# LMCache/LMCache

Measured on NVIDIA H100. Metric: kv_encode_decode_raw_GBps, higher is better.
Workload: dtype f32->u8 (bf16 KV)

## Files before the change

### lmcache_b200/csrc/codec.cu

```cuda
#include <cuda_bf16.h>
#include <cuda_fp16.h>
#include <cuda_runtime.h>
#include <stdint.h>
#include <stdlib.h>
#include <string.h>

#include <algorithm>
#include <vector>

#include "ac_core.cuh"
#include "common.cuh"

namespace b200kv {

constexpr int CT = 128;
constexpr int SPW = 6;
constexpr int SYMW = 43;
constexpr int PAIRW = 33;
constexpr int TEMPW_FUSED = 40;
constexpr int TEMPW_SPLIT = 132;
constexpr int TEMPW_FUSED_RANS = 48;
constexpr int CODER_AC = 0, CODER_RANS = 1;
constexpr int CODER_RANS_COMPACT = 2;
constexpr int kHdrRowWords = 8;
// ... 758 lines not shown
        const unsigned long long end = carry + wbase + inc;
        if (i < P.n_chunks) {
            const unsigned long long reserve = (end - start) * (unsigned long long)P.layers_left / (unsigned)P.nlay;
            const bool fits = (unsigned)i < fail0 && end + reserve <= (unsigned long long)P.arena_bytes;
            P.chunk_base[i] = fits ? end - v : ~0ull;
            if (fits) {
                P.ptotal[i] += P.totals[i];
                atomicMax(&s_end, end);
            } else {
                atomicOr(&P.err[i], 16u);
                atomicMin(&s_fail, (unsigned)i);
            }
        }
        __syncthreads();
        if (tid == 0) s_carry = s_end;
        __syncthreads();
    }
    if (tid == 0) {
        *P.cursor = s_carry;
        *P.fail_from = s_fail;
    }
    const int NLc = 2 * P.nlay;
    for (int k = tid; k < P.n_chunks * NLc; k += 1024) {
        const int j = k / NLc, pl = k - j * NLc;
        const uint32_t* tb = P.tile_tot + (int64_t)j * P.tiles_full;
        const unsigned long long off = tb[pl * P.tpp];
        const unsigned long long end = pl + 1 < NLc ? (unsigned long long)tb[(pl + 1) * P.tpp] : P.totals[j];
        const unsigned long long cb = P.chunk_base[j];
        int64_t* row = P.seg + ((int64_t)j * 2 * P.L + launch_plane(P, pl)) * 2;
        row[0] = cb == ~0ull ? -1 : (int64_t)(cb + off);
        row[1] = (int64_t)(end - off);
    }
}

__global__ void encl_init_kernel(EncParams P) {
    *P.cursor = 0ull;
    *P.fail_from = (unsigned)P.n_chunks;
}

__global__ void finalize_kernel(EncParams P) {
    const int j = blockIdx.x * blockDim.x + threadIdx.x;
    if (j >= P.n_chunks) return;
    const int t = chunk_tokens_of(P, j);
    const Layout lo = layout_of(P, t);
    b200kv_header* hd = reinterpret_cast<b200kv_header*>(P.out + (int64_t)j * P.out_stride);
    hd->magic = B200KV_MAGIC;
    hd->version = P.compact ? 3u : (uint32_t)P.coder + 1u;
    hd->L = P.L; hd->H = P.H; hd->D = P.D;
    hd->ntokens = t;
    hd->ngroups = lo.ngroups;
    hd->max_dtype = P.dtype;
    hd->payload_bytes = P.totals[j];
    hd->total_bytes = (uint64_t)lo.off_payload + P.totals[j];
    hd->status = P.err[j];
    hd->reserved[0] = hd->reserved[1] = hd->reserved[2] = 0u;
    if (P.sizes_out) P.sizes_out[j] = hd->status ? 0ull : hd->total_bytes;
    {
        uint8_t* c = reinterpret_cast<uint8_t*>(hd);
        const int64_t NL = 2 * (int64_t)P.L;
        const int64_t ends[3] = {lo.off_cdf + (P.compact ? NL : NL * P.C * kLp * 2), lo.off_maxes + NL * t * 2,
                                 lo.off_lengths + (int64_t)lo.ngroups * NL * P.C * (P.compact ? 1 : 4)};
        const int64_t starts[3] = {lo.off_maxes, lo.off_lengths, lo.off_payload};
        for (int k = 0; k < 3; ++k)
            for (int64_t b = ends[k]; b < starts[k]; ++b) c[b] = 0u;
    }
    if (P.compact) {
        uint8_t* nbmap = reinterpret_cast<uint8_t*>(hd) + lo.off_cdf;
        const int NL = 2 * P.L;
        for (int nl = 0; nl < (int)align16(NL); ++nl) nbmap[nl] = nl < NL ? (uint8_t)(2 * ((int)P.pt.maxq[nl] + 1)) : (uint8_t)0;
    }
}

struct DecChunk {
    const uint8_t* base;
    int64_t dst_tok;
    int32_t t, ngroups;
    uint32_t payload_bytes;
    int32_t ct0, ntw, cw0, cw1, dshift;
};

constexpr int kInlinePlanes = 128;
struct DecParams {
    PlaneTableT<kInlinePlanes> pt;
    const PlaneTable* gpt;
    int64_t sT, sH;
    const int64_t* slot_map;
    int32_t L, H, D, C, out_dtype, max_dtype, n_chunks, tpp, tiles_max;
    int32_t compact;
    int32_t lb, nlay;
    int32_t wtpp;
    const DecChunk* chunks;
    unsigned long long* tile_base;
    uint32_t* status;
};
static_assert(sizeof(DecParams) < kMaxParamBytes, "DecParams must stay under 4 KB of kernel parameters");

template <bool GT>
__device__ __forceinline__ const uint16_t* dec_plane(const DecParams& P, int nl) {
    if constexpr (GT) return P.gpt->p[nl];
    else return P.pt.p[nl];
}
template <bool GT>
__device__ __forceinline__ float dec_maxq(const DecParams& P, int nl) {
    if constexpr (GT) return P.gpt->maxq[nl];
    else return P.pt.maxq[nl];
}

__global__ void __launch_bounds__(128) tile_sum_kernel(DecParams P) {
    const int j = blockIdx.y;
    const int tile = blockIdx.x * 4 + (threadIdx.x >> 5);
    const int lane = threadIdx.x & 31;
    const DecChunk dc = P.chunks[j];
    const int NL = 2 * P.L;
    const int ntiles = dc.ngroups * NL * P.tpp;
    if (tile >= ntiles) return;
    const int plane_row = tile / P.tpp;
    const int ct = tile - plane_row * P.tpp;
    const Layout lo = layout_of(P, dc.t);
    const int c0 = ct * CT, c1 = min(P.C, c0 + CT);
    uint32_t s = 0;
    for (int c = c0 + lane; c < c1; c += 32) s += load_len(dc.base + lo.off_lengths, (int64_t)plane_row * P.C + c, P.compact != 0);
    s = __reduce_add_sync(0xffffffffu, s);
    if (lane == 0) P.tile_base[(int64_t)j * P.tiles_max + tile] = s;
}

__global__ void __launch_bounds__(1024) tile_scan_kernel(DecParams P) {
    __shared__ unsigned long long s_w[32];
    __shared__ unsigned long long s_carry;
    const int j = blockIdx.x;
    const DecChunk dc = P.chunks[j];
    const int ntiles = dc.ngroups * 2 * P.L * P.tpp;
    unsigned long long* tb = P.tile_base + (int64_t)j * P.tiles_max;
    const int lane = threadIdx.x & 31, wid = threadIdx.x >> 5;
    if (threadIdx.x == 0) s_carry = 0ull;
    __syncthreads();
    for (int base = 0; base < ntiles; base += 1024) {
        const int i = base + threadIdx.x;
        const unsigned long long v = i < ntiles ? tb[i] : 0ull;
        unsigned long long inc = v;
#pragma unroll
        for (int o = 1; o < 32; o <<= 1) {
            unsigned long long n = __shfl_up_sync(0xffffffffu, inc, o);
            if (lane >= o) inc += n;
        }
        if (lane == 31) s_w[wid] = inc;
        __syncthreads();
        unsigned long long wbase = 0ull, tot = 0ull;
        for (int w = 0; w < 32; ++w) {
            const unsigned long long s = s_w[w];
            if (w < wid) wbase += s;
            tot += s;
        }
        const unsigned long long carry = s_carry;
        if (i < ntiles) tb[i] = carry + wbase + inc - v;
        __syncthreads();
        if (threadIdx.x == 0) s_carry = carry + tot;
        __syncthreads();
    }
}

__global__ void __launch_bounds__(1024) plane_offsets_kernel(const uint8_t* base, int64_t stride, int64_t* out) {
    __shared__ uint32_t s_sum[B200KV_MAX_PLANES];
    const uint8_t* c = base + (int64_t)blockIdx.x * stride;
    int64_t* o = out + (int64_t)blockIdx.x * (B200KV_MAX_PLANES + 1);
    const uint32_t* hw = reinterpret_cast<const uint32_t*>(c);
    const uint32_t version = hw[1], L = hw[2], H = hw[3], D = hw[4], t = hw[5];
    const uint64_t total = *reinterpret_cast<const uint64_t*>(c + 40);
    const uint64_t C64 = (uint64_t)H * D;
    if (hw[0] != B200KV_MAGIC || version != 3u || L == 0u || 2u * L > (uint32_t)B200KV_MAX_PLANES || H == 0u || D == 0u ||
        t == 0u || t > (uint32_t)kGroup || C64 > (uint64_t)stride || C64 >= (1ull << 31)) {
        if (threadIdx.x == 0) o[0] = -1;
        return;
    }
    const int NL = 2 * (int)L;
    const int64_t C = (int64_t)C64;
    const Layout lo = make_layout((int)L, (int)C, (int)t, 1);
    if ((uint64_t)lo.off_payload > total || lo.off_payload > stride) {
        if (threadIdx.x == 0) o[0] = -1;
        return;
    }
    const uint8_t* half = c + lo.off_lengths;
    const int lane = threadIdx.x & 31, warp = threadIdx.x >> 5;
    for (int p = NL + 1 + (int)threadIdx.x; p <= B200KV_MAX_PLANES; p += blockDim.x) o[p] = 0;
    for (int p = warp; p < NL; p += blockDim.x >> 5) {
        const uint8_t* row = half + p * C;
        uint32_t sum = 0;
        if ((C & 15) == 0) {
            const uint4* v = reinterpret_cast<const uint4*>(row);
#pragma unroll 4
            for (int64_t i = lane; i < C / 16; i += 32) {
                const uint4 q = v[i];
                sum = __dp4a(q.x, 0x01010101u, sum);
                sum = __dp4a(q.y, 0x01010101u, sum);
                sum = __dp4a(q.z, 0x01010101u, sum);
                sum = __dp4a(q.w, 0x01010101u, sum);
            }
        } else {
            for (int64_t i = lane; i < C; i += 32) sum += row[i];
        }
        sum = __reduce_add_sync(0xffffffffu, sum);
        if (lane == 0) s_sum[p] = sum;
    }
    __syncthreads();
    if (threadIdx.x == 0) {
        int64_t off = lo.off_payload;
        o[0] = off;
        for (int p = 0; p < NL; ++p) {
            off += 2 * (int64_t)s_sum[p];
            o[p + 1] = off;
        }
        if (off != (int64_t)total) o[0] = -1;
    }
}

struct WordSrc {
    const uint32_t* base;
    uint32_t idx;
    uint32_t ahead;
    __device__ __forceinline__ void prime() { ahead = __ldg(base + idx); ++idx; }
    __device__ __forceinline__ uint32_t next_be() {
        const uint32_t w = ahead;
        ahead = __ldg(base + idx);
        ++idx;
        return __byte_perm(w, 0u, 0x0123);
    }
};

struct LeWordSrc {
    const uint32_t* p;
    __device__ __forceinline__ uint32_t next_le() { return __ldg(p++); }
};

__device__ __forceinline__ uint16_t out_half(float v, int dt) {
    return dt ? __half_as_ushort(__float2half_rn(v)) : __bfloat16_as_ushort(__float2bfloat16_rn(v));
}
template <int OUT_DT>
__device__ __forceinline__ void store_half(uint16_t* p, float v) {
    if constexpr (OUT_DT) *reinterpret_cast<__half*>(p) = __float2half_rn(v);
    else *reinterpret_cast<__nv_bfloat16*>(p) = __float2bfloat16_rn(v);
}

template <int OUT_DT>
__device__ __forceinline__ void store_dequant(uint16_t* base, uint32_t off, float lutv, float row_max, uint32_t two) {
    const float v = __fmul_rn(lutv, row_max);
    if constexpr (OUT_DT)
        asm volatile("{\n\t.reg .b64 ad;\n\t.reg .b32 r;\n\t.reg .b16 lo, hi;\n\t"
                     "mad.wide.u32 ad, %1, %3, %0;\n\t"
                     "cvt.rn.f16x2.f32 r, 0f00000000, %2;\n\t"
                     "mov.b32 {lo, hi}, r;\n\t"
                     "st.global.b16 [ad], lo;\n\t}" ::"l"(base), "r"(off), "f"(v), "r"(two) : "memory");
    else
        asm volatile("{\n\t.reg .b64 ad;\n\t.reg .b32 r;\n\t.reg .b16 lo, hi;\n\t"
                     "mad.wide.u32 ad, %1, %3, %0;\n\t"
                     "cvt.rn.bf16x2.f32 r, 0f00000000, %2;\n\t"
                     "mov.b32 {lo, hi}, r;\n\t"
                     "st.global.b16 [ad], lo;\n\t}" ::"l"(base), "r"(off), "f"(v), "r"(two) : "memory");
}

template <int OUT_DT, int NSTEPS, bool PAGED>
__device__ __forceinline__ void decode_stream(const uint8_t* cont, uint32_t my_off, const uint32_t* erow,
                                              const float* lut, const float* mx, uint16_t* dst, uint32_t sT, int gt,
                                              const int64_t* slots) {
    const uint32_t skip = my_off & 3u;
    WordSrc src{reinterpret_cast<const uint32_t*>(cont), my_off >> 2, 0u};
    src.prime();
    DecState2 st;
    dec_init2(st, src, skip);
    uint16_t* d = dst;
    auto lut_at = [&](uint32_t s4) { return *reinterpret_cast<const float*>(reinterpret_cast<const char*>(lut) + s4); };
    if constexpr (PAGED) {
        for (int i = 0; i < gt - 1; ++i)
            store_half<OUT_DT>(dst + __ldg(slots + i) * (int64_t)sT,
                               dequant_value(lut_at(dec_symbol2<NSTEPS>(st, src, erow, false)), mx[i]));
        store_half<OUT_DT>(dst + __ldg(slots + gt - 1) * (int64_t)sT,
                           dequant_value(lut_at(dec_symbol2<NSTEPS>(st, src, erow, true)), mx[gt - 1]));
    } else {
        for (int i = 0; i < gt - 1; ++i, d += sT)
            store_half<OUT_DT>(d, dequant_value(lut_at(dec_symbol2<NSTEPS>(st, src, erow, false)), mx[i]));
        store_half<OUT_DT>(d, dequant_value(lut_at(dec_symbol2<NSTEPS>(st, src, erow, true)), mx[gt - 1]));
    }
}

template <uint32_t ROWS, uint32_t PITCH>
__device__ __forceinline__ void rans_search_step(uint32_t& a, uint32_t key, uint32_t one) {
    uint32_t ev;
    asm volatile("ld.shared.u32 %0, [%1+%2];" : "=r"(ev) : "r"(a), "n"(ROWS * PITCH));
    asm("{\n\t.reg .pred p;\n\tsetp.le.u32 p, %1, %2;\n\t@p mad.lo.u32 %0, %3, %4, %0;\n\t}"
        : "+r"(a) : "r"(ev), "r"(key), "r"(one), "n"(ROWS * PITCH));
}

template <int OUT_DT, int NSTEPS, bool PAGED, bool TR>
__device__ __forceinline__ uint32_t rans_decode_stream(const uint8_t* cont, uint32_t my_off, const uint32_t* pk,
                                                       const float* lut, const float* mx, uint16_t* dst, uint32_t sT, int gt,
                                                       const int64_t* slots, uint32_t one) {
    const uint32_t* const wbase = reinterpret_cast<const uint32_t*>(cont);
    uint32_t idx = my_off >> 2;
    struct Src {
        const uint32_t* b; uint32_t& i;
        __device__ __forceinline__ uint32_t next_le() { return __ldg(b + i++); }
    } src{wbase, idx};
    RansDec st;
    rans_dec_init(st, src, (my_off >> 1) & 1u);
    constexpr uint32_t H = 1u << (NSTEPS - 1);
    constexpr uint32_t kPitch = TR ? CT * 4u : 4u;
    constexpr uint32_t kIdx = TR ? CT : 1u;
    const uint32_t a0 = (uint32_t)__cvta_generic_to_shared(pk);
    const uint32_t a0h = a0 + kPitch * H;
    const uint32_t r_mid = pk[kIdx * H], r_lo = pk[kIdx * (H / 2)], r_hi = pk[kIdx * (H + H / 2)];
    const uint32_t lut_a = (uint32_t)__cvta_generic_to_shared(lut);
    const uint32_t lut_rel = lut_a - a0;
    uint32_t off = 0u;
    const uint32_t c64k = one << 16, mone = 0u - one, two = one + one, c25 = one << 25;
    auto step = [&](float row_max, int i) {
        uint32_t key, xh;
        asm("mad.lo.u32 %0, %1, %2, 65535;" : "=r"(key) : "r"(st.x), "r"(c64k));
        asm("mul.hi.u32 %0, %1, %2;" : "=r"(xh) : "r"(st.x), "r"(c64k));
        const bool p1 = r_mid <= key;
        uint32_t a = p1 ? a0h : a0;
        const uint32_t m = p1 ? r_hi : r_lo;
        asm("{\n\t.reg .pred p;\n\tsetp.le.u32 p, %1, %2;\n\t@p mad.lo.u32 %0, %3, %4, %0;\n\t}"
            : "+r"(a) : "r"(m), "r"(key), "r"(one), "n"(kPitch * (H / 2)));
        if constexpr (H >= 16) rans_search_step<4, kPitch>(a, key, one);
        rans_search_step<2, kPitch>(a, key, one);
        rans_search_step<1, kPitch>(a, key, one);
        uint32_t e, la;
        float lv;
        asm volatile("ld.shared.u32 %0, [%1];" : "=r"(e) : "r"(a));
        if constexpr (TR) asm("mad.hi.u32 %0, %1, %2, %3;" : "=r"(la) : "r"(a - a0), "r"(c25), "r"(lut_a));
        else la = a + lut_rel;
        asm volatile("ld.shared.f32 %0, [%1];" : "=f"(lv) : "r"(la));
        uint32_t dl;
        asm("mul.hi.u32 %0, %1, %2;" : "=r"(dl) : "r"(key - e), "r"(c64k));
        st.x = (e & 0xffffu) * xh + dl;
        const uint32_t* const wad = wbase + idx;
        asm volatile(
            "{\n\t.reg .pred p, q;\n\t"
            "setp.lt.u32 p, %0, 65536;\n\t"
            "setp.eq.and.u32 q, %3, 0x1076, p;\n\t"
            "@p prmt.b32 %0, %0, %1, %3;\n\t"
            "@p mad.lo.u32 %3, %3, %7, 0x20ca;\n\t"
            "@q mov.b32 %1, %2;\n\t"
            "@q ld.global.nc.u32 %2, [%5];\n\t"
            "@q mad.lo.u32 %4, %6, %6, %4;\n\t"
            "}"
            : "+r"(st.x), "+r"(st.cur), "+r"(st.nxt), "+r"(st.sel), "+r"(idx)
            : "l"(wad), "r"(one), "r"(mone));
        if constexpr (PAGED) {
            store_dequant<OUT_DT>(dst + __ldg(slots + i) * (int64_t)sT, 0u, lv, row_max, two);
        } else {
            store_dequant<OUT_DT>(dst, off, lv, row_max, two);
            asm("mad.lo.u32 %0, %1, %2, %0;" : "+r"(off) : "r"(one), "r"(sT));
        }
    };
    int i = 0;
#pragma unroll 1
    for (; i + 4 <= gt; i += 4) {
        const float4 m4 = *reinterpret_cast<const float4*>(mx + i);
        step(m4.x, i); step(m4.y, i + 1); step(m4.z, i + 2); step(m4.w, i + 3);
    }
#pragma unroll 1
    for (; i < gt; ++i) step(mx[i], i);
    return st.x;
}

template <int OUT_DT, bool PAGED, int CODER, bool TR, bool GT>
__global__ void __launch_bounds__(CT, 12) decode_kernel(DecParams P) {
    extern __shared__ __align__(128) uint32_t smem[];
    uint32_t* tab = smem;
    float* mx = reinterpret_cast<float*>(smem + CT * kLp);
    float* lut = mx + kGroup;
    __shared__ uint32_t s_warp[CT / 32];

    const int tid = threadIdx.x;
    const int j = blockIdx.y;
    const DecChunk dc = P.chunks[j];
    const int NL = 2 * P.L;
    const int per_group = NL * P.tpp;
    const int launch_group = 2 * P.nlay * P.wtpp;
    const int g = blockIdx.x / launch_group;
    if (g >= dc.ngroups) return;
    const int kt = blockIdx.x - g * launch_group;
    const int kp = kt / P.wtpp;
    const int wt = kt - kp * P.wtpp;
    if (wt >= dc.ntw) return;
    const int nl = kp + (kp < P.nlay ? P.lb : P.L - P.nlay + P.lb);
    const int ct = dc.ct0 + wt;
    const int tile = g * per_group + nl * P.tpp + ct;
    const int tok0 = g * kGroup;
    const int gt = min(kGroup, dc.t - tok0);
    const int c = ct * CT + tid;
    const bool in_c = c < P.C;
    const bool active = c >= dc.cw0 && c < dc.cw1;
    const int ncols = min(CT, P.C - ct * CT);
    const Layout lo = layout_of(P, dc.t);

    const uint32_t len = in_c ? load_len(dc.base + lo.off_lengths, ((int64_t)g * NL + nl) * P.C + c, P.compact != 0) : 0u;
    uint32_t tile_total;
    const uint32_t my_rel = block_excl_scan(len, s_warp, &tile_total);
    const unsigned long long want = P.tile_base[(int64_t)j * P.tiles_max + tile] + my_rel;
    const bool beyond = want + len > (unsigned long long)dc.payload_bytes;
    const uint32_t my_off = (uint32_t)lo.off_payload + (uint32_t)min(want, (unsigned long long)dc.payload_bytes);

    const uint16_t* cdf_src = reinterpret_cast<const uint16_t*>(dc.base + lo.off_cdf) + ((int64_t)nl * P.C + ct * CT) * kLp;
    const uint16_t* maxes = reinterpret_cast<const uint16_t*>(dc.base + lo.off_maxes) + (int64_t)nl * dc.t + tok0;
    const float cq = dec_maxq<GT>(P, nl);
    bool built = false;
    uint32_t hl = 0u;
    if constexpr (CODER == CODER_RANS) {
        if (P.compact) {
            float* pn = mx;
            const float tf = (float)dc.t;
            for (int n = tid; n <= kGroup; n += CT) pn[n] = fdiv((float)n, tf);
            __syncthreads();
            const int nb = 2 * ((int)cq + 1);
            const uint32_t mbytes = (uint32_t)hdr_mask_bytes(nb);
            const uint8_t* sp = dc.base + my_off;
            const uint32_t al = (uint32_t)(reinterpret_cast<uintptr_t>(sp) & 3u);
            const uint32_t* wp = reinterpret_cast<const uint32_t*>(sp - al);
            const uint32_t fs = 8u * al;
            uint32_t x_prev = __ldg(wp), x_next = __ldg(wp + 1);
            const uint32_t hb0 = __funnelshift_r(x_prev, x_next, fs);
            uint32_t mask = hb0;
            if (nb <= 8) mask &= 0xffu;
            else if (nb <= 16) mask &= 0xffffu;
            if (nb < 32) mask &= (1u << nb) - 1u;
            hl = hdr_len(mask, nb);
            const uint32_t top = 0x80000000u >> __clz((int)mask);
            const bool all_short = __popc(__ballot_sync(0xffffffffu, active && hl > 8u)) < 8;
            const uint32_t wany = __reduce_or_sync(0xffffffffu, active ? mask : 0u);
            if (active) {
                uint32_t sum = 0u;
                uint32_t hb[9];
                uint32_t widx = mbytes >> 2, inw = mbytes & 3u, cur = 0u;
                const uint8_t* const cb = sp + mbytes;
                if (!all_short) {
                    hb[0] = hb0;
#pragma unroll
                    for (int k = 1; k < 9; ++k) {
                        hb[k] = 0u;
                        if ((uint32_t)(4 * k) < hl && (k < 5 || nb > 16)) {
                            x_prev = x_next;
                            x_next = __ldg(wp + k + 1);
                            hb[k] = __funnelshift_r(x_prev, x_next, fs);
                        }
                    }
                    cur = (widx == 0u ? hb[0] : hb[1]) >> (8u * inw);
                }
                auto next_byte = [&]() -> uint32_t {
                    const uint32_t v = cur & 255u;
                    cur >>= 8;
                    if (++inw == 4u) {
                        inw = 0u;
                        ++widx;
                        cur = hb[1];
#pragma unroll
                        for (int k = 2; k < 9; ++k) cur = widx == (uint32_t)k ? hb[k] : cur;
                    }
                    return v;
                };
                auto count = [&](int i) -> uint32_t {
                    if (i >= nb) return 0u;
                    const uint32_t bit = 1u << (i & 31);
                    uint32_t n = 0u;
                    if (all_short) {
                        const uint32_t below = i == 0 ? 0u : mask & (0xffffffffu >> (32 - (i & 31)));
                        const uint32_t v = __ldg(cb + __popc(below));
                        n = (mask & bit) ? v : 0u;
                        n = (top & bit) ? (uint32_t)dc.t - sum : n;
                        sum += n;
                    } else if (mask & bit) {
                        n = (top & bit) ? (uint32_t)dc.t - sum : next_byte();
                        sum += n;
                    }
                    return min(n, (uint32_t)kGroup);
                };
                CdfAccum2 acc;
                acc.init();
                uint32_t c0 = 0u;
                const int nsearch = cq <= 7.0f ? 16 : 32;
#pragma unroll
                for (int i = 0; i < 32; ++i) {
                    if (i < nsearch) {
                        if ((wany >> i) & 1u) acc.absorb(pn[count(i)]);
                        uint32_t c1 = acc.value((uint32_t)i + 1u);
                        if (i == 31) c1 = 0x10000u;
                        const uint32_t e = rans_table_entry(c0, c1);
                        if (TR) tab[i * CT + tid] = e;
                        else tab[tid * kLp + i] = e;
                        c0 = c1;
                    }
                }
            }
            __syncthreads();
            for (int i = tid; i < gt; i += CT) mx[i] = half_to_float(maxes[i], P.max_dtype);
            if (tid < 32) lut[tid] = dequant_lut((uint32_t)tid, cq);
            built = true;
        }
    }
    if (!built) {
        if constexpr (CODER == CODER_RANS && TR) {
            uint16_t* stg = reinterpret_cast<uint16_t*>(smem) + (CT * kLp);
            for (int e = tid; e < ncols * kLp; e += CT) stg[e] = __ldg(cdf_src + e);
            for (int i = tid; i < gt; i += CT) mx[i] = half_to_float(maxes[i], P.max_dtype);
            if (tid < 32) lut[tid] = dequant_lut((uint32_t)tid, cq);
            __syncthreads();
            const uint16_t* my = stg + tid * kLp;
            if (active) {
                uint32_t c0 = my[0];
    #pragma unroll
                for (int i = 0; i < 16; ++i) {
                    const uint32_t c1 = my[i + 1];
                    tab[i * CT + tid] = rans_table_entry(c0, c1);
                    c0 = c1;
                }
            }
            if (cq > 7.0f) {
                uint32_t cv[17];
                if (active) {
    #pragma unroll
                    for (int i = 0; i < 16; ++i) cv[i] = my[16 + i];
                    cv[16] = 0x10000u;
                }
                __syncthreads();
                if (active) {
    #pragma unroll
                    for (int i = 0; i < 16; ++i) tab[(16 + i) * CT + tid] = rans_table_entry(cv[i], cv[i + 1]);
                }
            }
        } else {
            for (int e = tid; e < ncols * kLp; e += CT) {
                const uint32_t i = (uint32_t)e % (uint32_t)kLp;
                const uint32_t c0 = __ldg(cdf_src + e);
                if constexpr (CODER == CODER_RANS) {
                    const uint32_t c1 = i < 31u ? (uint32_t)__ldg(cdf_src + e + 1) : 0x10000u;
                    tab[e] = i < 32u ? rans_table_entry(c0, c1) : 0xFFFFFFFFu;
                } else {
                    tab[e] = dec_table_entry(i, c0);
                }
            }
            for (int i = tid; i < gt; i += CT) mx[i] = half_to_float(maxes[i], P.max_dtype);
            if (tid < 32) lut[tid] = dequant_lut((uint32_t)tid, cq);
        }
    }
    __syncthreads();

    if (!active) return;
    const uint32_t* erow = tab + tid * kLp;
    const int oc = c + dc.dshift;
    const int h = oc / P.D;
    uint16_t* dst = const_cast<uint16_t*>(dec_plane<GT>(P, nl)) + (PAGED ? 0 : (dc.dst_tok + tok0) * P.sT) + (int64_t)h * P.sH +
                    (oc - h * P.D);
    const int64_t* slots = PAGED ? P.slot_map + dc.dst_tok + tok0 : nullptr;
    uint32_t bad = beyond ? 2u : 0u;
    if constexpr (CODER == CODER_RANS) {
        uint32_t xf;
        const uint32_t one = min((uint32_t)P.n_chunks, 1u);
        const uint32_t* pk = TR ? tab + tid : tab + tid * kLp;
        if (cq <= 7.0f) xf = rans_decode_stream<OUT_DT, 4, PAGED, TR>(dc.base, my_off + hl, pk, lut, mx, dst, (uint32_t)P.sT, gt, slots, one);
        else xf = rans_decode_stream<OUT_DT, 5, PAGED, TR>(dc.base, my_off + hl, pk, lut, mx, dst, (uint32_t)P.sT, gt, slots, one);
        bad |= xf != kRansLow ? 1u : 0u;
    } else {
        if (cq <= 7.0f) decode_stream<OUT_DT, 4, PAGED>(dc.base, my_off, erow, lut, mx, dst, (uint32_t)P.sT, gt, slots);
        else decode_stream<OUT_DT, 5, PAGED>(dc.base, my_off, erow, lut, mx, dst, (uint32_t)P.sT, gt, slots);
    }
    if (bad != 0u && P.status != nullptr) atomicOr(&P.status[j], bad);
}

int make_plane_table(const b200kv_kv_desc* kv, const float* key_bins, const float* value_bins, PlaneTable* out) {
    B2_REQUIRE(kv != nullptr, "kv descriptor is NULL");
    B2_REQUIRE(kv->L > 0 && 2 * kv->L <= B200KV_MAX_PLANES, "L out of range");
    B2_REQUIRE(kv->H > 0 && kv->D > 0, "H/D must be positive");
    B2_REQUIRE(kv->dtype == B200KV_DT_BF16 || kv->dtype == B200KV_DT_FP16, "dtype must be bf16 or fp16");
    B2_REQUIRE(kv->planes != nullptr || kv->base != nullptr, "no KV pointer");
    for (int kvi = 0; kvi < 2; ++kvi)
        for (int l = 0; l < kv->L; ++l) {
            const int nl = kvi * kv->L + l;
            const uint16_t* p = kv->planes ? static_cast<const uint16_t*>(kv->planes[nl])
                                           : static_cast<const uint16_t*>(kv->base) + l * kv->sL + kvi * kv->sKV;
            B2_REQUIRE(p != nullptr, "NULL plane pointer");
            out->p[nl] = p;
            const float bins = kvi ? value_bins[l] : key_bins[l];
            out->maxq[nl] = floorf(bins / 2.0f) - 1.0f;
            B2_REQUIRE(out->maxq[nl] >= 1.0f && out->maxq[nl] <= 15.0f, "bins must be in [4, 32]");
        }
    return 0;
}

static int tiles_per_plane(int C) { return (C + CT - 1) / CT; }

enum { kProfAbsmax = 0, kProfCdf, kProfEncode, kProfFinalize, kProfTileSum, kProfTileScan, kProfDecode, kProfCount };
static bool g_prof_on = false;
static cudaEvent_t g_prof_ev[kProfCount][2];
static bool g_prof_have[kProfCount];
static bool g_prof_init = false;

struct ProfScope {
    int slot;
    cudaStream_t stream;
    ProfScope(int slot_, cudaStream_t s) : slot(slot_), stream(s) {
        if (!g_prof_on) return;
        if (!g_prof_init) {
            for (int i = 0; i < kProfCount; ++i) { cudaEventCreate(&g_prof_ev[i][0]); cudaEventCreate(&g_prof_ev[i][1]); }
            g_prof_init = true;
        }
        cudaEventRecord(g_prof_ev[slot][0], stream);
    }
    ~ProfScope() {
        if (!g_prof_on) return;
        cudaEventRecord(g_prof_ev[slot][1], stream);
        g_prof_have[slot] = true;
    }
};

static int enc_tempw(bool fused, int coder, bool compact = false) {
    if (compact) return TEMPW_FUSED_RANS_HDR;
    return fused ? (coder == CODER_RANS ? TEMPW_FUSED_RANS : TEMPW_FUSED) : TEMPW_SPLIT;
}

static size_t enc_ws_layout(int64_t n_tiles_alloc, int n_chunks, int tempw, int coder, bool compact, size_t* off_tot,
                            size_t* off_totals, size_t* off_err, size_t* off_state, size_t* off_temp) {
    size_t o = 0;
    *off_tot = o;    o += (size_t)n_tiles_alloc * 4;  o = (o + 255) & ~(size_t)255;
    *off_totals = o; o += (size_t)n_chunks * 8;       o = (o + 255) & ~(size_t)255;
    *off_err = o;    o += (size_t)n_chunks * 4;       o = (o + 255) & ~(size_t)255;
    *off_state = o;  o += coder == CODER_RANS ? (size_t)n_tiles_alloc * CT * (compact ? 16 : 4) : 0;  o = (o + 255) & ~(size_t)255;
    *off_temp = o;   o += (size_t)n_tiles_alloc * CT * (size_t)tempw * 4;
    return (o + 255) & ~(size_t)255;
}

struct EnclWs { size_t err, ptotal, cbase, state, tot, totals, rstate, temp, bytes; };
static EnclWs encl_ws_layout(int n_chunks, int64_t call_tiles) {
    EnclWs w;
    size_t o = 0;
    auto take = [&](size_t* off, size_t n) { *off = o; o = (o + n + 255) & ~(size_t)255; };
    take(&w.err, (size_t)n_chunks * 4);
    take(&w.ptotal, (size_t)n_chunks * 8);
    take(&w.cbase, (size_t)n_chunks * 8);
    take(&w.state, 16);
    take(&w.tot, (size_t)call_tiles * 4);
    take(&w.totals, (size_t)n_chunks * 8);
    take(&w.rstate, (size_t)call_tiles * CT * 16);
    take(&w.temp, (size_t)call_tiles * CT * TEMPW_FUSED_RANS_HDR * 4);
    w.bytes = o;
    return w;
}

constexpr uint32_t kEncPlanMagic = 0x4e4c5045u;
struct LayerSet {
    static constexpr int kWords = B200KV_MAX_PLANES / 2 / 64;
    uint64_t w[kWords];
    static LayerSet range(int a, int b) {
        LayerSet s;
        for (int i = 0; i < kWords; ++i) {
            const int lo = std::max(a - 64 * i, 0), hi = std::min(b - 64 * i, 64);
            s.w[i] = lo >= hi ? 0ull : (hi - lo == 64 ? ~0ull : ((1ull << (hi - lo)) - 1ull) << lo);
        }
        return s;
    }
    bool intersects(const LayerSet& o) const {
        uint64_t x = 0ull;
        for (int i = 0; i < kWords; ++i) x |= w[i] & o.w[i];
        return x != 0ull;
    }
    bool operator==(const LayerSet& o) const {
        for (int i = 0; i < kWords; ++i)
            if (w[i] != o.w[i]) return false;
        return true;
    }
    void add(const LayerSet& o) {
        for (int i = 0; i < kWords; ++i) w[i] |= o.w[i];
    }
    int count() const {
        int n = 0;
        for (int i = 0; i < kWords; ++i) n += __builtin_popcountll(w[i]);
        return n;
    }
};
static_assert(LayerSet::kWords * 64 == B200KV_MAX_PLANES / 2, "one bit per layer");
struct EncPlan {
    uint32_t magic;
    int32_t max_layers;
    LayerSet done;
    EncParams P;
};
static_assert(sizeof(EncPlan) <= sizeof(b200kv_encode_plan_t), "b200kv_encode_plan_t too small");

constexpr size_t kSmemFused = (size_t)(((CT * SYMW + (CT * kLp * 2 + 3) / 4 + 3) & ~3) + kGroup + 8) * 4;
constexpr int kStageRans = 12 * 1024;

static int launch_absmax(const EncParams& P, const b200kv_kv_desc* kv, int64_t total_tokens, cudaStream_t stream) {
    bool vec = (kv->D % 8 == 0) && (kv->sT % 8 == 0) && (kv->sH % 8 == 0);
    for (int nl = 0; nl < 2 * P.L && vec; ++nl) vec = (reinterpret_cast<uintptr_t>(P.pt.p[nl]) & 15) == 0;
    const bool paged = P.slot_map != nullptr;
    const int64_t rows = 2 * (int64_t)P.nlay * total_tokens;
    const int64_t blocks = (rows + 7) / 8;
    B2_REQUIRE(blocks < (1ll << 31), "too many rows in one call");
    if (vec && !paged) absmax_kernel<true, false><<<(unsigned)blocks, 256, 0, stream>>>(P, total_tokens);
    else if (vec) absmax_kernel<true, true><<<(unsigned)blocks, 256, 0, stream>>>(P, total_tokens);
    else if (!paged) absmax_kernel<false, false><<<(unsigned)blocks, 256, 0, stream>>>(P, total_tokens);
    else absmax_kernel<false, true><<<(unsigned)blocks, 256, 0, stream>>>(P, total_tokens);
    B2_CHECK_CUDA(cudaGetLastError());
    return 0;
}

static size_t dec_ws_layout(int64_t tiles_max, int n_chunks, int L, size_t* off_tb, size_t* off_pt) {
    size_t o = ((size_t)n_chunks * sizeof(DecChunk) + 255) & ~(size_t)255;
    *off_tb = o;
    o += (size_t)n_chunks * (size_t)tiles_max * 8;
    o = (o + 255) & ~(size_t)255;
    *off_pt = o;
    if (2 * L > kInlinePlanes) o = (o + sizeof(PlaneTable) + 255) & ~(size_t)255;
    return o;
}

constexpr uint32_t kPlanMagic = 0x4e4c5044u;
struct DecPlan {
    uint32_t magic;
    int32_t coder;
    int32_t transposed;
    int32_t gmax;
    DecParams P;
};
static_assert(sizeof(DecPlan) <= sizeof(b200kv_decode_plan_t), "b200kv_decode_plan_t too small");

}

using namespace b200kv;

extern "C" {

int b200kv_container_layout(int32_t L, int32_t H, int32_t D, int32_t ntokens, b200kv_layout* out) {
    return b200kv_container_layout_v(L, H, D, ntokens, CODER_RANS, out);
}

int b200kv_container_layout_v(int32_t L, int32_t H, int32_t D, int32_t ntokens, int32_t coder, b200kv_layout* out) {
    B2_REQUIRE(out != nullptr && L > 0 && H > 0 && D > 0 && ntokens > 0, "bad shape");
    B2_REQUIRE(coder >= CODER_AC && coder <= CODER_RANS_COMPACT, "unknown coder");
    const int compact = coder == CODER_RANS_COMPACT ? 1 : 0;
    B2_REQUIRE(!compact || ntokens <= kGroup, "the compact container holds chunks of at most 256 tokens");
    const Layout lo = make_layout(L, H * D, ntokens, compact);
    out->off_cdf = lo.off_cdf;
    out->off_maxes = lo.off_maxes;
    out->off_lengths = lo.off_lengths;
    out->off_payload = lo.off_payload;
    out->fixed_bytes = lo.off_payload;
    const int64_t streams = 2 * (int64_t)L * H * D;
    out->max_total_bytes = align16(lo.off_payload + streams * (2 * (int64_t)ntokens + 4 * (int64_t)lo.ngroups +
                                                              (compact ? kHdrMax : 0)) + 16);
    return 0;
}

int b200kv_plane_offsets(const void* container, int64_t nbytes, int64_t* out, int32_t n_out) {
    B2_REQUIRE(container != nullptr && out != nullptr && nbytes >= (int64_t)sizeof(b200kv_header), "bad arguments");
    b200kv_header hd;
    memcpy(&hd, container, sizeof(hd));
    B2_REQUIRE(hd.magic == B200KV_MAGIC && hd.version == 3, "not a version-3 container");
    B2_REQUIRE(hd.L > 0 && 2 * (int64_t)hd.L <= B200KV_MAX_PLANES && hd.H > 0 && hd.D > 0 && hd.ntokens > 0 &&
               hd.ntokens <= (uint32_t)kGroup, "impossible shape");
    const int NL = 2 * (int)hd.L;
    const int64_t C = (int64_t)hd.H * hd.D;
    B2_REQUIRE(n_out >= NL + 1, "out must hold 2L + 1 offsets");
    const Layout lo = make_layout((int)hd.L, (int)C, (int)hd.ntokens, 1);
    B2_REQUIRE(nbytes >= lo.off_payload, "buffer shorter than the fixed sections");
    const uint8_t* half = static_cast<const uint8_t*>(container) + lo.off_lengths;
    int64_t o = lo.off_payload;
    out[0] = o;
    for (int p = 0; p < NL; ++p) {
        uint32_t sum = 0;
        for (int64_t c = 0; c < C; ++c) sum += half[p * C + c];
        o += 2 * (int64_t)sum;
        out[p + 1] = o;
    }
    return o == (int64_t)hd.total_bytes ? 0 : 1;
}

int b200kv_plane_offsets_device(const void* containers, int64_t stride, int32_t n, int64_t* out, void* stream) {
    B2_REQUIRE(containers != nullptr && out != nullptr && n > 0 && stride >= (int64_t)sizeof(b200kv_header) &&
               (stride & 15) == 0 && (reinterpret_cast<uintptr_t>(containers) & 15) == 0, "bad arguments");
    plane_offsets_kernel<<<(unsigned)n, 1024, 0, static_cast<cudaStream_t>(stream)>>>(static_cast<const uint8_t*>(containers),
                                                                                      stride, out);
    B2_CHECK_CUDA(cudaGetLastError());
    return 0;
}

int64_t b200kv_encode_workspace_bytes(int32_t L, int32_t H, int32_t D, int32_t chunk_tokens, int32_t n_chunks,
                                      int32_t coder) {
    if (L <= 0 || H <= 0 || D <= 0 || chunk_tokens <= 0 || n_chunks <= 0) return -2;
    coder &= 0xff;
    const bool compact = coder == CODER_RANS_COMPACT;
    if (compact) coder = CODER_RANS;
    if (coder != CODER_AC && coder != CODER_RANS) return -2;
    if (compact && chunk_tokens > kGroup) return -2;
    const int64_t G = (chunk_tokens + kGroup - 1) / kGroup;
    const int64_t n_tiles = (int64_t)n_chunks * G * 2 * L * tiles_per_plane(H * D);
    size_t a, b, c, d, e;
    return (int64_t)enc_ws_layout(n_tiles, n_chunks, enc_tempw(chunk_tokens <= kGroup, coder, compact), coder, compact, &a, &b, &c, &d, &e);
}

int64_t b200kv_decode_workspace_bytes(int32_t L, int32_t H, int32_t D, int32_t chunk_tokens, int32_t n_chunks) {
    if (L <= 0 || H <= 0 || D <= 0 || chunk_tokens <= 0 || n_chunks <= 0) return -2;
    const int64_t G = (chunk_tokens + kGroup - 1) / kGroup;
    const int64_t tiles_max = G * 2 * L * tiles_per_plane(H * D);
    size_t a, b;
    return (int64_t)dec_ws_layout(tiles_max, n_chunks, L, &a, &b);
}

int b200kv_encode_chunks(const b200kv_kv_desc* kv, int64_t tok_begin, int32_t n_chunks, int32_t chunk_tokens,
                         int32_t last_chunk_tokens, const float* key_bins, const float* value_bins, int32_t coder,
                         void* out, int64_t out_stride, uint64_t* sizes_out, void* workspace, int64_t workspace_bytes,
                         void* stream_) {
    cudaStream_t stream = static_cast<cudaStream_t>(stream_);
    EncParams P;
    B2_REQUIRE(key_bins && value_bins, "bins are NULL");
    const bool hint_mid = (coder & B200KV_ENCODE_HINT_MID_ENTROPY) != 0;
    coder &= 0xff;
    B2_REQUIRE(coder >= CODER_AC && coder <= CODER_RANS_COMPACT, "coder must be one of B200KV_CODER_*");
    P.compact = coder == CODER_RANS_COMPACT ? 1 : 0;
    if (P.compact) coder = CODER_RANS;
    P.coder = coder;
    if (int rc = make_plane_table(kv, key_bins, value_bins, &P.pt)) return rc;
    B2_REQUIRE(n_chunks > 0 && chunk_tokens > 0, "n_chunks / chunk_tokens must be positive");
    B2_REQUIRE(!P.compact || chunk_tokens <= kGroup, "the compact container (B200KV_CODER_RANS_COMPACT) holds chunks of at most 256 tokens");
    B2_REQUIRE(last_chunk_tokens > 0 && last_chunk_tokens <= chunk_tokens, "last_chunk_tokens out of range");
    B2_REQUIRE(out != nullptr && (reinterpret_cast<uintptr_t>(out) & 15) == 0 && (out_stride & 15) == 0,
               "out / out_stride must be 16-byte aligned");
    B2_REQUIRE(tok_begin >= 0, "tok_begin must be >= 0");
    P.sT = kv->sT; P.sH = kv->sH; P.tok_begin = tok_begin;
    P.slot_map = kv->slot_map;
    const bool paged = kv->slot_map != nullptr;
    P.L = kv->L; P.H = kv->H; P.D = kv->D; P.C = kv->H * kv->D; P.dtype = kv->dtype;
    P.n_chunks = n_chunks; P.chunk_tokens = chunk_tokens; P.last_chunk_tokens = last_chunk_tokens;
    P.tpp = tiles_per_plane(P.C);
    P.out = static_cast<uint8_t*>(out);
    P.out_stride = out_stride;
    P.sizes_out = sizes_out;
    P.lb = 0; P.nlay = P.L;
    P.arena = nullptr; P.arena_bytes = 0; P.chunk_base = nullptr; P.cursor = nullptr; P.fail_from = nullptr;
    P.ptotal = nullptr; P.seg = nullptr; P.layers_left = 0;
    const Layout lo = make_layout(P.L, P.C, chunk_tokens, P.compact);
    B2_REQUIRE(out_stride >= lo.off_payload + 16, "out_stride smaller than the fixed container sections");

    const int64_t G = lo.ngroups;
    const int64_t per_group = 2 * (int64_t)P.L * P.tpp;
    const int64_t tiles_full = G * per_group;
    const int64_t n_tiles = (int64_t)n_chunks * tiles_full;
    const bool fused = chunk_tokens <= kGroup;
    P.tiles_full = (int32_t)tiles_full;
    P.tempw = enc_tempw(fused, coder, P.compact != 0);
    size_t off_tot, off_totals, off_err, off_state, off_temp;
    const size_t need = enc_ws_layout(n_tiles, n_chunks, P.tempw, coder, P.compact != 0, &off_tot, &off_totals, &off_err, &off_state,
                                      &off_temp);
    B2_REQUIRE(workspace != nullptr && workspace_bytes >= (int64_t)need, "workspace too small");
    B2_REQUIRE(n_tiles < (1ll << 31) && tiles_full < (1ll << 31), "too many tiles in one call");
    uint8_t* ws = static_cast<uint8_t*>(workspace);
    P.tile_tot = reinterpret_cast<uint32_t*>(ws + off_tot);
    P.totals = reinterpret_cast<unsigned long long*>(ws + off_totals);
    P.err = reinterpret_cast<unsigned int*>(ws + off_err);
    P.temp = reinterpret_cast<uint32_t*>(ws + off_temp);
    P.rstate = reinterpret_cast<uint32_t*>(ws + off_state);
    B2_CHECK_CUDA(cudaMemsetAsync(ws, 0, off_state, stream));

    const int64_t total_tokens = (int64_t)(n_chunks - 1) * chunk_tokens + last_chunk_tokens;
// ... 416 lines not shown
```

Measured before the change: 388.1.

## Compact rANS decode tables to present symbols and use shallower per-warp search

```diff
diff --git a/lmcache_b200/csrc/codec.cu b/lmcache_b200/csrc/codec.cu
--- a/lmcache_b200/csrc/codec.cu
+++ b/lmcache_b200/csrc/codec.cu
@@ -1084,6 +1084,7 @@
     RansDec st;
     rans_dec_init(st, src, (my_off >> 1) & 1u);
     constexpr uint32_t H = 1u << (NSTEPS - 1);
+    constexpr bool kCompact = TR && NSTEPS < 5;
     constexpr uint32_t kPitch = TR ? CT * 4u : 4u;
     constexpr uint32_t kIdx = TR ? CT : 1u;
     const uint32_t a0 = (uint32_t)__cvta_generic_to_shared(pk);
@@ -1103,14 +1104,19 @@
         asm("{\n\t.reg .pred p;\n\tsetp.le.u32 p, %1, %2;\n\t@p mad.lo.u32 %0, %3, %4, %0;\n\t}"
             : "+r"(a) : "r"(m), "r"(key), "r"(one), "n"(kPitch * (H / 2)));
         if constexpr (H >= 16) rans_search_step<4, kPitch>(a, key, one);
-        rans_search_step<2, kPitch>(a, key, one);
-        rans_search_step<1, kPitch>(a, key, one);
-        uint32_t e, la;
+        if constexpr (H >= 8) rans_search_step<2, kPitch>(a, key, one);
+        if constexpr (H >= 4) rans_search_step<1, kPitch>(a, key, one);
+        uint32_t e;
         float lv;
         asm volatile("ld.shared.u32 %0, [%1];" : "=r"(e) : "r"(a));
-        if constexpr (TR) asm("mad.hi.u32 %0, %1, %2, %3;" : "=r"(la) : "r"(a - a0), "r"(c25), "r"(lut_a));
-        else la = a + lut_rel;
-        asm volatile("ld.shared.f32 %0, [%1];" : "=f"(lv) : "r"(la));
+        if constexpr (kCompact) {
+            asm volatile("ld.shared.f32 %0, [%1+%2];" : "=f"(lv) : "r"(a), "n"(16u * kPitch));
+        } else {
+            uint32_t la;
+            if constexpr (TR) asm("mad.hi.u32 %0, %1, %2, %3;" : "=r"(la) : "r"(a - a0), "r"(c25), "r"(lut_a));
+            else la = a + lut_rel;
+            asm volatile("ld.shared.f32 %0, [%1];" : "=f"(lv) : "r"(la));
+        }
         uint32_t dl;
         asm("mul.hi.u32 %0, %1, %2;" : "=r"(dl) : "r"(key - e), "r"(c64k));
         st.x = (e & 0xffffu) * xh + dl;
@@ -1186,8 +1192,13 @@
     const uint16_t* cdf_src = reinterpret_cast<const uint16_t*>(dc.base + lo.off_cdf) + ((int64_t)nl * P.C + ct * CT) * kLp;
     const uint16_t* maxes = reinterpret_cast<const uint16_t*>(dc.base + lo.off_maxes) + (int64_t)nl * dc.t + tok0;
     const float cq = dec_maxq<GT>(P, nl);
-    bool built = false;
     uint32_t hl = 0u;
+    uint32_t pm = 0u;
+    int wsteps = cq <= 7.0f ? 4 : 5;
+    auto depth_of = [&](uint32_t my_pm) {
+        const uint32_t kmax = __reduce_max_sync(0xffffffffu, (uint32_t)__popc(my_pm));
+        return kmax <= 4u ? 2 : kmax <= 8u ? 3 : kmax <= 16u ? 4 : 5;
+    };
     if constexpr (CODER == CODER_RANS) {
         if (P.compact) {
             float* pn = mx;
@@ -1210,6 +1221,8 @@
             const uint32_t top = 0x80000000u >> __clz((int)mask);
             const bool all_short = __popc(__ballot_sync(0xffffffffu, active && hl > 8u)) < 8;
             const uint32_t wany = __reduce_or_sync(0xffffffffu, active ? mask : 0u);
+            pm = active ? mask : 0u;
+            if (TR) wsteps = depth_of(pm);
             if (active) {
                 uint32_t sum = 0u;
                 uint32_t hb[9];
@@ -1258,7 +1271,7 @@
                 };
                 CdfAccum2 acc;
                 acc.init();
-                uint32_t c0 = 0u;
+                uint32_t c0 = 0u, pos = 0u;
                 const int nsearch = cq <= 7.0f ? 16 : 32;
 #pragma unroll
                 for (int i = 0; i < 32; ++i) {
@@ -1267,8 +1280,9 @@
                         uint32_t c1 = acc.value((uint32_t)i + 1u);
                         if (i == 31) c1 = 0x10000u;
                         const uint32_t e = rans_table_entry(c0, c1);
-                        if (TR) tab[i * CT + tid] = e;
-                        else tab[tid * kLp + i] = e;
+                        if (!TR) tab[tid * kLp + i] = e;
+                        else if (wsteps == 5) tab[i * CT + tid] = e;
+                        else if ((mask >> i) & 1u) tab[pos++ * CT + tid] = e;
                         c0 = c1;
                     }
                 }
@@ -1276,57 +1290,85 @@
             __syncthreads();
             for (int i = tid; i < gt; i += CT) mx[i] = half_to_float(maxes[i], P.max_dtype);
             if (tid < 32) lut[tid] = dequant_lut((uint32_t)tid, cq);
-            built = true;
-        }
-    }
-    if (!built) {
-        if constexpr (CODER == CODER_RANS && TR) {
+        } else if (!TR) {
+            for (int e = tid; e < ncols * kLp; e += CT) {
+                const uint32_t i = (uint32_t)e % (uint32_t)kLp;
+                const uint32_t c0 = __ldg(cdf_src + e);
+                const uint32_t c1 = i < 31u ? (uint32_t)__ldg(cdf_src + e + 1) : 0x10000u;
+                tab[e] = i < 32u ? rans_table_entry(c0, c1) : 0xFFFFFFFFu;
+            }
+            for (int i = tid; i < gt; i += CT) mx[i] = half_to_float(maxes[i], P.max_dtype);
+            if (tid < 32) lut[tid] = dequant_lut((uint32_t)tid, cq);
+        } else {
             uint16_t* stg = reinterpret_cast<uint16_t*>(smem) + (CT * kLp);
             for (int e = tid; e < ncols * kLp; e += CT) stg[e] = __ldg(cdf_src + e);
             for (int i = tid; i < gt; i += CT) mx[i] = half_to_float(maxes[i], P.max_dtype);
             if (tid < 32) lut[tid] = dequant_lut((uint32_t)tid, cq);
             __syncthreads();
             const uint16_t* my = stg + tid * kLp;
+            const bool wide = cq > 7.0f;
+            if (active) {
+#pragma unroll
+                for (int i = 0; i < 32; ++i) {
+                    if (i < 16 || wide) {
+                        const uint32_t c1 = i == 31 ? 0x10000u : (uint32_t)my[i + 1];
+                        pm |= ((c1 - my[i]) & 0xffffu) >= 2u ? 1u << i : 0u;
+                    }
+                }
+            }
+            wsteps = depth_of(pm);
+            uint32_t pos = 0u, cv[17];
             if (active) {
                 uint32_t c0 = my[0];
-    #pragma unroll
+#pragma unroll
                 for (int i = 0; i < 16; ++i) {
                     const uint32_t c1 = my[i + 1];
-                    tab[i * CT + tid] = rans_table_entry(c0, c1);
+                    const uint32_t e = rans_table_entry(c0, c1);
+                    if (wsteps == 5) tab[i * CT + tid] = e;
+                    else if ((pm >> i) & 1u) tab[pos++ * CT + tid] = e;
                     c0 = c1;
                 }
-            }
-            if (cq > 7.0f) {
-                uint32_t cv[17];
-                if (active) {
-    #pragma unroll
+                if (wide) {
+#pragma unroll
                     for (int i = 0; i < 16; ++i) cv[i] = my[16 + i];
                     cv[16] = 0x10000u;
                 }
+            }
+            if (wide) {
                 __syncthreads();
                 if (active) {
-    #pragma unroll
-                    for (int i = 0; i < 16; ++i) tab[(16 + i) * CT + tid] = rans_table_entry(cv[i], cv[i + 1]);
+#pragma unroll
+                    for (int i = 0; i < 16; ++i) {
+                        const uint32_t e = rans_table_entry(cv[i], cv[i + 1]);
+                        if (wsteps == 5) tab[(16 + i) * CT + tid] = e;
+                        else if ((pm >> (16 + i)) & 1u) tab[pos++ * CT + tid] = e;
+                    }
                 }
             }
-        } else {
-            for (int e = tid; e < ncols * kLp; e += CT) {
-                const uint32_t i = (uint32_t)e % (uint32_t)kLp;
-                const uint32_t c0 = __ldg(cdf_src + e);
-                if constexpr (CODER == CODER_RANS) {
-                    const uint32_t c1 = i < 31u ? (uint32_t)__ldg(cdf_src + e + 1) : 0x10000u;
-                    tab[e] = i < 32u ? rans_table_entry(c0, c1) : 0xFFFFFFFFu;
-                } else {
-                    tab[e] = dec_table_entry(i, c0);
-                }
-            }
-            for (int i = tid; i < gt; i += CT) mx[i] = half_to_float(maxes[i], P.max_dtype);
-            if (tid < 32) lut[tid] = dequant_lut((uint32_t)tid, cq);
-        }
+        }
+    } else {
+        for (int e = tid; e < ncols * kLp; e += CT) {
+            const uint32_t i = (uint32_t)e % (uint32_t)kLp;
+            tab[e] = dec_table_entry(i, __ldg(cdf_src + e));
+        }
+        for (int i = tid; i < gt; i += CT) mx[i] = half_to_float(maxes[i], P.max_dtype);
+        if (tid < 32) lut[tid] = dequant_lut((uint32_t)tid, cq);
     }
     __syncthreads();
 
     if (!active) return;
+    if (CODER == CODER_RANS && TR && wsteps < 5) {
+        uint32_t pos = 0u, e = 0u, v = 0u;
+        for (uint32_t m = pm; m != 0u; m &= m - 1u, ++pos) {
+            v = __float_as_uint(lut[__ffs((int)m) - 1]);
+            tab[(16u + pos) * CT + tid] = v;
+        }
+        if (pos != 0u) e = tab[(pos - 1u) * CT + tid];
+        for (; pos < (1u << wsteps); ++pos) {
+            tab[pos * CT + tid] = e;
+            tab[(16u + pos) * CT + tid] = v;
+        }
+    }
     const uint32_t* erow = tab + tid * kLp;
     const int oc = c + dc.dshift;
     const int h = oc / P.D;
@@ -1337,9 +1379,13 @@
     if constexpr (CODER == CODER_RANS) {
         uint32_t xf;
         const uint32_t one = min((uint32_t)P.n_chunks, 1u);
-        const uint32_t* pk = TR ? tab + tid : tab + tid * kLp;
-        if (cq <= 7.0f) xf = rans_decode_stream<OUT_DT, 4, PAGED, TR>(dc.base, my_off + hl, pk, lut, mx, dst, (uint32_t)P.sT, gt, slots, one);
-        else xf = rans_decode_stream<OUT_DT, 5, PAGED, TR>(dc.base, my_off + hl, pk, lut, mx, dst, (uint32_t)P.sT, gt, slots, one);
+        const uint32_t* pk = TR ? tab + tid : erow;
+        const uint8_t* b = dc.base;
+        const uint32_t so = my_off + hl, sT = (uint32_t)P.sT;
+        if (TR && wsteps == 2) xf = rans_decode_stream<OUT_DT, 2, PAGED, TR>(b, so, pk, lut, mx, dst, sT, gt, slots, one);
+        else if (TR && wsteps == 3) xf = rans_decode_stream<OUT_DT, 3, PAGED, TR>(b, so, pk, lut, mx, dst, sT, gt, slots, one);
+        else if (wsteps == 4) xf = rans_decode_stream<OUT_DT, 4, PAGED, TR>(b, so, pk, lut, mx, dst, sT, gt, slots, one);
+        else xf = rans_decode_stream<OUT_DT, 5, PAGED, TR>(b, so, pk, lut, mx, dst, sT, gt, slots, one);
         bad |= xf != kRansLow ? 1u : 0u;
     } else {
         if (cq <= 7.0f) decode_stream<OUT_DT, 4, PAGED>(dc.base, my_off, erow, lut, mx, dst, (uint32_t)P.sT, gt, slots);
```

Result: slower. 384.1 (median of 6 runs) (-1.0%).
